# streamer45/streamkit

Hardware: AMD Instinct MI355X
Metric: real-time factor (audio-sec/wall-sec) Whisper-small Oneshot batch (higher is better)
Workload: dtype f16; 1 GPU; Whisper-small Oneshot batch, 64x30 s synthetic 16 kHz clips per GPU (configs[1]), greedy T=0 with the temperature ladder armed, random-init weights in GGML f16 container; precision=f16_mfma: f16 operands on v_mfma_f32_16x16x32_f16, f32 accumulate, clips_per_gpu=64, fallback_requested=0

## Files before the change

streamkit_amd/csrc/skw_kernels_f16.hip:

```cpp
#include "skw_dev_common.h"
#include <algorithm>
#include <atomic>
#include <type_traits>

typedef _Float16 f16x8 __attribute__((ext_vector_type(8)));
#ifndef SKW_VOCAB_W_AUX
#define SKW_VOCAB_W_AUX 0
#endif
#ifndef SKW_EPI_ST_NT
#define SKW_EPI_ST_NT 0
#endif
#ifndef SKW_EPI_RES_NT
#define SKW_EPI_RES_NT 0
#endif
#ifndef SKW_DEC_W_AUX
#define SKW_DEC_W_AUX 0
#endif
#define MFMA16X32(a, b, c) __builtin_amdgcn_mfma_f32_16x16x32_f16((a), (b), (c), 0, 0, 0)

typedef __attribute__((address_space(1))) const void* gptr_t;
typedef __attribute__((address_space(3))) void* lptr_t;

__device__ __forceinline__ int inv_kperm32(int p) { return ((p & 7) << 2) | ((p >> 3) & 3); }
template <int EPI> struct Epi16 {
// ... 105 lines not shown
            int gn = n0 + c; if (gn > a.N - 1) gn = a.N - 1;
            gB[i] = a.W + (long)gn * a.ldw + pchunk * 8;
        }
    };
    auto stage = [&](int buf, int kb) {
        char* base = lds + buf * (BM + BN) * 128;
        if (PROBE && (a.probe & 32)) {
#pragma unroll
            for (int i = 0; i < A_PIECES; ++i) __builtin_amdgcn_global_load_lds((gptr_t)(gA[i] + kb * 64), (lptr_t)(base + (wave * A_PIECES + i) * 1024), 16, 0, 2);
        } else {
#pragma unroll
            for (int i = 0; i < A_PIECES; ++i) __builtin_amdgcn_global_load_lds((gptr_t)(gA[i] + kb * 64), (lptr_t)(base + (wave * A_PIECES + i) * 1024), 16, 0, 0);
        }
        if (PROBE && (a.probe & 64)) {
#pragma unroll
            for (int i = 0; i < B_PIECES; ++i) __builtin_amdgcn_global_load_lds((gptr_t)(gB[i] + kb * 64), (lptr_t)(base + BM * 128 + (wave * B_PIECES + i) * 1024), 16, 0, 2);
        } else {
#pragma unroll
            for (int i = 0; i < B_PIECES; ++i) __builtin_amdgcn_global_load_lds((gptr_t)(gB[i] + kb * 64), (lptr_t)(base + BM * 128 + (wave * B_PIECES + i) * 1024), 16, 0, 0);
        }
    };
    const int fo0 = ((g ^ (r16 & 7)) << 4), fo1 = fo0 ^ 64;
    const int aoff = (wr * WTM + r16) * 128, boff = BM * 128 + (wc * WTN + r16) * 128;
    const int xoff = X_IS_M ? aoff : boff, yoff = X_IS_M ? boff : aoff;
    const int nk = a.K >> 6;
    const int x_lim = X_IS_M ? Mv : a.N, y_lim = X_IS_M ? a.N : a.M;
    int tile = blockIdx.x;
    if (tile >= nblk) return;
    int m0, n0; tile_origin(tile, m0, n0); tile_sources(m0, n0);
    stage(0, 0);
    for (;;) {
        asm volatile("s_waitcnt vmcnt(0)" ::: "memory");
        __syncthreads();
        f32x4 acc[TX][TY];
#pragma unroll
        for (int i = 0; i < TX; ++i)
#pragma unroll
            for (int j = 0; j < TY; ++j) acc[i][j] = (f32x4){0.f, 0.f, 0.f, 0.f};
        for (int kb = 0; kb < nk; ++kb) {
            const char* base = lds + (kb & 1) * (BM + BN) * 128;
            if (!PROBE) stage((kb + 1) & 1, min(kb + 1, nk - 1));
            else if (kb + 1 < nk && !(a.probe & 1)) stage((kb + 1) & 1, kb + 1);
#pragma unroll
            for (int kk = 0; kk < 2; ++kk) {
                if (PROBE && (a.probe & 2)) break;
                const int fo = kk ? fo1 : fo0;
                f16x8 fx[TX], fy[TY];
#pragma unroll
                for (int t = 0; t < TX; ++t) fx[t] = *(const f16x8*)(base + xoff + t * 2048 + fo);
#pragma unroll
                for (int t = 0; t < TY; ++t) fy[t] = *(const f16x8*)(base + yoff + t * 2048 + fo);
#pragma unroll
                for (int i = 0; i < TX; ++i)
#pragma unroll
                    for (int j = 0; j < TY; ++j) acc[i][j] = MFMA16X32(fx[i], fy[j], acc[i][j]);
            }
            if (kb + 1 < nk) { asm volatile("s_waitcnt vmcnt(0)" ::: "memory"); __syncthreads(); }
        }
        if (!PROBE) asm volatile("s_waitcnt vmcnt(0)" ::: "memory");
        __syncthreads();
        const int X0 = X_IS_M ? m0 : n0, Y0 = X_IS_M ? n0 : m0;
        tile += gridDim.x;
        const bool more = tile < nblk;
        if (more) { tile_origin(tile, m0, n0); tile_sources(m0, n0); if (!(PROBE && (a.probe & 1))) stage(0, 0); }
        if (!(PROBE && (a.probe & 4))) {
            constexpr bool F32OUT = Epi16Out<EPI>::F32OUT;
            constexpr int BX = X_IS_M ? BM : BN, BY = X_IS_M ? BN : BM, WTX = X_IS_M ? WTM : WTN, WTY = X_IS_M ? WTN : WTM;
            constexpr int ESZ = F32OUT ? 4 : 2, ROWB = BX * ESZ, CPR = ROWB / 16;
            constexpr int RP = ((BM + BN) * 128) / ROWB < BY ? ((BM + BN) * 128) / ROWB : BY;
            constexpr int NPASS = BY / RP, CE = 16 / ESZ;
            static_assert(BY % RP == 0 && (CPR & (CPR - 1)) == 0, "whole passes, power-of-two chunks per row");
            char* stg = lds + (BM + BN) * 128;
            float* bias_l = (float*)(lds + 2 * (BM + BN) * 128);
            const int wX = X_IS_M ? wr : wc, wY = X_IS_M ? wc : wr;
            const int div = X_IS_M ? a.Tpad : (a.n_ctx > 0 ? a.n_ctx : 1), org = X_IS_M ? X0 : Y0;
            const int qb = org / div, rb = org % div;
            {
                constexpr int NB = X_IS_M ? BY : BX;
                if (tid < NB) { const int pos = (X_IS_M ? Y0 : X0) + tid; const int f = (PERM && !X_IS_M) ? ((pos & ~31) | inv_kperm32(pos & 31)) : pos;
                bias_l[tid] = (a.bias && f < a.N) ? a.bias[f] : 0.0f; }
                __syncthreads();
            }
            for (int pass = 0; pass < NPASS; ++pass) {
                auto phase_a = [&](auto raw_tag) {
                    constexpr bool RAW = decltype(raw_tag)::value;
#pragma unroll
                for (int j = 0; j < TY; ++j) {
                    const int yl = wY * WTY + j * 16 + r16;
                    if ((wY * WTY + j * 16) / RP != pass) continue;
                    const int ylp = yl - pass * RP;
#pragma unroll
                    for (int i = 0; i < TX; ++i) {
                        const int xl = wX * WTX + i * 16 + 4 * g, p0 = X0 + xl;
                        float o[4];
                        const f32x4 bx = X_IS_M ? (f32x4){bias_l[yl], bias_l[yl], bias_l[yl], bias_l[yl]} : *(const f32x4*)(bias_l + xl);
#pragma unroll
                        for (int r = 0; r < 4; ++r) {
                            o[r] = RAW ? acc[i][j][r] : epi_value<EPI>(a, p0 + r, acc[i][j][r], bx[r]);
                            if (X_IS_M) { int key = rb + (((xl + r) & ~31) | inv_kperm32((xl + r) & 31)); if (key >= a.Tpad) key -= a.Tpad; if (key >= a.n_ctx) o[r] = 0.0f; }
                        }
                        const int ck = xl / CE;
                        char* dst = stg + ylp * ROWB + ((ck ^ (ylp & (CPR - 1))) << 4);
                        if (F32OUT) *(f32x4*)dst = (f32x4){o[0], o[1], o[2], o[3]};
                        else *(f16x4*)(dst + ((xl % CE) >= 4 ? 8 : 0)) = (f16x4){f2h(o[0]), f2h(o[1]), f2h(o[2]), f2h(o[3])};
                    }
                }
                };
                if (PROBE && (a.probe & 16)) phase_a(std::true_type{}); else phase_a(std::false_type{});
                __syncthreads();
                constexpr int NCH = RP * CPR / (NW * 64), BATCH = !F32OUT ? 2 : (NCH < 4 ? NCH : 4);
                static_assert((RP * CPR) % (NW * 64) == 0 && NCH % BATCH == 0, "whole chunks per thread");
#pragma unroll 1
                for (int c0 = 0; c0 < NCH; c0 += BATCH) {
                    long off[BATCH]; f32x4 opnd[BATCH]; int lofs[BATCH];
#pragma unroll
                    for (int u = 0; u < BATCH; ++u) {
                        const int cid = tid + (c0 + u) * NW * 64, ylp = cid / CPR, pc = cid % CPR, ck = pc ^ (ylp & (CPR - 1));
                        const int y = Y0 + pass * RP + ylp, px = X0 + ck * CE;
                        lofs[u] = ylp * ROWB + (pc << 4);
                        off[u] = (y >= y_lim || px >= x_lim || (PROBE && (a.probe & 8))) ? -1 : epi_chunk_offset<EPI>(a, y, px, pass * RP + ylp, ck * CE, qb, rb);
                        if (EPI == EPI_F32) opnd[u] = (a.res && off[u] >= 0) ? (SKW_EPI_RES_NT ? __builtin_nontemporal_load((const f32x4*)(a.res + (long)y * a.ldres + px))
                                                                                                : *(const f32x4*)(a.res + (long)y * a.ldres + px))
                                                                              : (f32x4){0.f, 0.f, 0.f, 0.f};
                        if (EPI == EPI_CONV2) { int i = rb + pass * RP + ylp; if (i >= a.n_ctx) i -= a.n_ctx;
                        opnd[u] = (off[u] >= 0) ? *(const f32x4*)(a.pe + (long)i * a.N + px) : (f32x4){0.f, 0.f, 0.f, 0.f}; }
                    }
#pragma unroll
                    for (int u = 0; u < BATCH; ++u) {
                        if (off[u] < 0) continue;
                        if (F32OUT) {
                            f32x4 v = *(const f32x4*)(stg + lofs[u]);
                            if (EPI == EPI_F32) { if (a.res) { v[0] = v[0] + opnd[u][0]; v[1] = v[1] + opnd[u][1]; v[2] = v[2] + opnd[u][2]; v[3] = v[3] + opnd[u][3]; } }
                            else { v[0] = opnd[u][0] + v[0]; v[1] = opnd[u][1] + v[1]; v[2] = opnd[u][2] + v[2]; v[3] = opnd[u][3] + v[3]; }
                            if (SKW_EPI_ST_NT) __builtin_nontemporal_store(v, (f32x4*)((float*)a.C + off[u])); else *(f32x4*)((float*)a.C + off[u]) = v;
                        } else { const u32x4 o16 = *(const u32x4*)(stg + lofs[u]); if (SKW_EPI_ST_NT) __builtin_nontemporal_store(o16, (u32x4*)((half_t*)a.C + off[u]));
                        else *(u32x4*)((half_t*)a.C + off[u]) = o16; }
                    }
                }
                __syncthreads();
            }
        }
        if (!more) break;
    }
}

static int skw_cur_device() { int dev = 0; if (hipGetDevice(&dev) != hipSuccess || dev < 0 || dev >= 64) dev = 0; return dev; }
static int skw_cu_count() {
    static std::atomic<int> n[64];
    const int dev = skw_cur_device(); int v = n[dev].load(std::memory_order_relaxed);
    if (!v) { hipDeviceProp_t p; v = (hipGetDeviceProperties(&p, dev) == hipSuccess && p.multiProcessorCount > 0) ? p.multiProcessorCount : 256; n[dev].store(v, std::memory_order_relaxed); }
    return v;
}
#define SKW_LDS_BARRIER() asm volatile("s_waitcnt lgkmcnt(0)\n\ts_barrier" ::: "memory")
template <int EPI, bool PROBE = false>
__global__ __launch_bounds__(256, 2) void k_gemm16w(SkwGemmArgs a) {
    constexpr int BM = 128, BN = 256, NW = 4, WTN = 64, TMT = BM / 16, TNT = WTN / 16, SLOT = BM * 128, NSLOT = 3, PARK = 32768;
    constexpr bool X_IS_M = Epi16<EPI>::X_IS_M, PERM = Epi16<EPI>::PERM;
    constexpr int TX = X_IS_M ? TMT : TNT, TY = X_IS_M ? TNT : TMT;
    constexpr int A_PIECES = BM / 8 / NW;
    __shared__ __attribute__((aligned(1024))) char lds[65536];
    const int tid = threadIdx.x, lane = tid & 63, wave = __builtin_amdgcn_readfirstlane(tid >> 6);
    const int Mv = X_IS_M ? (a.M / a.n_ctx) * a.Tpad : a.M;
    const int nbn = (a.N + BN - 1) / BN, nbm = (Mv + BM - 1) / BM, nblk = nbn * nbm;
    const int r16 = lane & 15, g = lane >> 4;
    const int prow = lane >> 3, pchunk = (lane & 7) ^ prow;
    const int nk = a.K >> 6, nk32 = a.K >> 5, nstrip = a.N >> 4;
    const half_t* gA[A_PIECES];
    unsigned woff[TNT];
    const int ng = a.wgroups > 1 ? a.wgroups : 1, ngn = nbn / ng, mparts = 8 / ng, mp = (nbm + mparts - 1) / mparts;
    const int nwalk = ng > 1 ? 8 * mp * ngn : nblk;
    auto tile_origin = [&](int tile, int& m0, int& n0) {
        if (ng > 1) {
            const int x = tile & 7, y = tile >> 3, gsel = x % ng, part = x / ng;
            const int m = part * mp + y / ngn;
            m0 = m < min(nbm, (part + 1) * mp) ? m * BM : -1; n0 = (gsel * ngn + y % ngn) * BN;
            return;
        }
        int q = nblk >> 3, r = nblk & 7, x = tile & 7, y = tile >> 3;
        const int bid = (x < r ? x * (q + 1) : r * (q + 1) + (x - r) * q) + y;
        m0 = (bid / nbn) * BM; n0 = (bid % nbn) * BN;
    };
    auto tile_sources = [&](int m0, int n0) {
#pragma unroll
        for (int i = 0; i < A_PIECES; ++i) {
            int c = (wave * A_PIECES + i) * 8 + prow; if (X_IS_M && PERM) c = (c & ~31) | inv_kperm32(c & 31);
            int gm = m0 + c;
            if (PROBE && (a.probe & 32768)) gm = c;
            if (X_IS_M) { const int b = gm / a.Tpad, key = gm % a.Tpad; gm = min(b, a.M / a.n_ctx - 1) * a.n_ctx + min(key, a.n_ctx - 1); }
            if (gm > a.M - 1) gm = a.M - 1;
            const long off = a.a_rows_per_batch ? (long)(gm / a.a_rows_per_batch) * a.a_batch_stride + (long)(gm % a.a_rows_per_batch) * a.lda : (long)gm * a.lda;
            gA[i] = a.A + off + pchunk * 8;
        }
#pragma unroll
        for (int t = 0; t < TNT; ++t) {
            int s = (n0 + wave * WTN + 16 * t) >> 4; if (s > nstrip - 1) s = nstrip - 1;
            woff[t] = (unsigned)(s * nk32) * 1024u + lane * 16;
        }
    };
    auto stage = [&](int slot, int kb) {
        char* base = lds + slot * SLOT;
#pragma unroll
        for (int i = 0; i < A_PIECES; ++i) __builtin_amdgcn_global_load_lds((gptr_t)(gA[i] + kb * 64), (lptr_t)(base + (wave * A_PIECES + i) * 1024), 16, 0, 0);
    };
    auto loadw = [&](f16x8 (&w)[TNT], int kb32) {
#pragma unroll
        for (int t = 0; t < TNT; ++t) asm volatile("global_load_dwordx4 %0, %1, %2" : "=v"(w[t]) : "v"(woff[t] + (unsigned)kb32 * 1024u), "s"(a.Wf) : "memory");
    };
    const int fo0 = ((g ^ (r16 & 7)) << 4), fo1 = fo0 ^ 64;
    const int aoff = r16 * 128;
    const int x_lim = X_IS_M ? Mv : a.N, y_lim = X_IS_M ? a.N : a.M;
    constexpr int BIAS_OFF = NSLOT * SLOT, BIAS_MAX = (65536 - BIAS_OFF) / 4;
    const bool bias_lds = a.N <= BIAS_MAX;
    if (bias_lds) {
        float* bl = (float*)(lds + BIAS_OFF);
        for (int p = tid; p < a.N; p += 256) { const int f = (PERM && !X_IS_M) ? ((p & ~31) | inv_kperm32(p & 31)) : p; bl[p] = a.bias ? a.bias[f] : 0.0f; }
        SKW_LDS_BARRIER();
    }
    for (int tile = blockIdx.x; tile < nwalk; tile += gridDim.x) {
        int m0, n0; tile_origin(tile, m0, n0);
        if (m0 < 0) continue;
        tile_sources(m0, n0);
        f16x8 w0[TNT], w1[TNT];
        stage(0, 0);
        stage(1, min(1, nk - 1));
        loadw(w0, 0);
        stage(2, min(2, nk - 1));
        loadw(w1, 1);
        f32x4 acc[TX][TY];
#pragma unroll
        for (int i = 0; i < TX; ++i)
#pragma unroll
            for (int j = 0; j < TY; ++j) acc[i][j] = (f32x4){0.f, 0.f, 0.f, 0.f};
        asm volatile("s_waitcnt vmcnt(16)" ::: "memory");
        __builtin_amdgcn_s_barrier();
        f16x8 lo[4], hi[4];
        auto rd = [&](f16x8 (&f)[4], const char* base, int t0, int fo) {
#pragma unroll
            for (int t = 0; t < 4; ++t) f[t] = *(const f16x8*)(base + aoff + (t0 + t) * 2048 + fo);
        };
        auto mm = [&](const f16x8 (&f)[4], const f16x8 (&w)[TNT], int t0, f16x8 (&nf)[4], const char* nb, int nt0, int nfo) {
            if (PROBE && (a.probe & 4096)) { asm volatile("" :: "v"(f[0]), "v"(f[3]), "v"(w[0])); rd(nf, nb, nt0, nfo); return; }
#pragma unroll
            for (int t = 0; t < 4; ++t)
#pragma unroll
                for (int q = 0; q < TNT; ++q) {
                    if (X_IS_M) acc[t0 + t][q] = MFMA16X32(f[t], w[q], acc[t0 + t][q]);
                    else acc[q][t0 + t] = MFMA16X32(w[q], f[t], acc[q][t0 + t]);
                    if (t == 0 && q == 0) { __builtin_amdgcn_sched_barrier(0); rd(nf, nb, nt0, nfo); __builtin_amdgcn_sched_barrier(0); }
                }
        };
        rd(lo, lds, 0, fo0);
        for (int kb = 0; kb < nk; ++kb) {
            const char* base = lds + (kb % NSLOT) * SLOT;
            const char* nbase = lds + ((kb + 1) % NSLOT) * SLOT;
            asm volatile("s_waitcnt vmcnt(8)" : "+v"(w0[0]), "+v"(w0[1]), "+v"(w0[2]), "+v"(w0[3]) :: "memory");
            mm(lo, w0, 0, hi, base, 4, fo0);
            __builtin_amdgcn_sched_barrier(0);
            mm(hi, w0, 4, lo, base, 0, fo1);
            if (!(PROBE && (a.probe & 8192))) loadw(w0, min(2 * kb + 2, nk32 - 1));
            __builtin_amdgcn_sched_barrier(0);
            asm volatile("s_waitcnt vmcnt(4)" : "+v"(w1[0]), "+v"(w1[1]), "+v"(w1[2]), "+v"(w1[3]) :: "memory");
            mm(lo, w1, 0, hi, base, 4, fo1);
            __builtin_amdgcn_sched_barrier(0);
            asm volatile("s_waitcnt lgkmcnt(0)\n\ts_barrier" : "+v"(hi[0]), "+v"(hi[1]), "+v"(hi[2]), "+v"(hi[3]) :: "memory");
            if (!(PROBE && (a.probe & 16384))) stage(kb % NSLOT, min(kb + 3, nk - 1));
            mm(hi, w1, 4, lo, nbase, 0, fo0);
            if (!(PROBE && (a.probe & 8192))) loadw(w1, min(2 * kb + 3, nk32 - 1));
            __builtin_amdgcn_sched_barrier(0);
        }
        asm volatile("" :: "v"(lo[0]), "v"(lo[1]), "v"(lo[2]), "v"(lo[3]));
        asm volatile("s_waitcnt vmcnt(0)" : "+v"(w0[0]), "+v"(w0[1]), "+v"(w0[2]), "+v"(w0[3]), "+v"(w1[0]), "+v"(w1[1]), "+v"(w1[2]), "+v"(w1[3]) :: "memory");
        __syncthreads();
        const int X0 = X_IS_M ? m0 : n0, Y0 = X_IS_M ? n0 : m0;
        if (PROBE && (a.probe & 1024)) { asm volatile("" :: "v"(acc[0][0]), "v"(acc[TX - 1][TY - 1])); }
        else {
            constexpr bool F32OUT = Epi16Out<EPI>::F32OUT;
            constexpr int ESZ = F32OUT ? 4 : 2, CE = 16 / ESZ;
            constexpr int WX = X_IS_M ? BM : WTN, WY = X_IS_M ? WTN : BM;
            constexpr int RB = WX * ESZ, CPRW = RB / 16;
            constexpr int FILLB = 8192;
            constexpr int RH = FILLB / RB < WY ? FILLB / RB : WY, NFILL = WY / RH;
            constexpr int NCH = RH * CPRW / 64, TYF = RH / 16;
            static_assert(WY % RH == 0 && (RH * CPRW) % 64 == 0 && RH % 16 == 0, "whole fills");
            char* wl = lds + wave * FILLB;
            const int xw = X_IS_M ? 0 : wave * WTN, yw = X_IS_M ? wave * WTN : 0;
            const int div = X_IS_M ? a.Tpad : (a.n_ctx > 0 ? a.n_ctx : 1), org = X_IS_M ? X0 : Y0;
            const int qb = org / div, rb = org % div;
            constexpr bool FASTOFF = (EPI == EPI_HEADS_F16);
            const bool interior = FASTOFF && Y0 + BM <= y_lim && X0 + BN <= x_lim && rb + BM <= div;
            const bool has_pad = X_IS_M && (rb + BM > a.n_ctx);
            f32x4 bx[X_IS_M ? 1 : TX]; float by[X_IS_M ? TY : 1];
            const float* bl = (const float*)(lds + BIAS_OFF);
            if (!X_IS_M) {
#pragma unroll
                for (int i = 0; i < TX; ++i) {
                    const int p0 = X0 + xw + i * 16 + 4 * g;
                    if (bias_lds) bx[i] = (p0 < a.N) ? *(const f32x4*)(bl + p0) : (f32x4){0.f, 0.f, 0.f, 0.f};
                    else {
#pragma unroll
                        for (int r = 0; r < 4; ++r) { const int pos = p0 + r, f = PERM ? ((pos & ~31) | inv_kperm32(pos & 31)) : pos; bx[i][r] = (a.bias && f < a.N) ? a.bias[f] : 0.0f; }
                    }
                }
            } else {
#pragma unroll
                for (int j = 0; j < TY; ++j) { const int f = Y0 + yw + j * 16 + r16; by[j] = (f < a.N) ? (bias_lds ? bl[f] : (a.bias ? a.bias[f] : 0.0f)) : 0.0f; }
            }
#pragma unroll
            for (int fill = 0; fill < NFILL; ++fill) {
                f32x4 opnd[F32OUT ? NCH : 1];
                if (F32OUT) {
#pragma unroll
                    for (int u = 0; u < NCH; ++u) {
                        const int cid = lane + 64 * u, rho = cid / CPRW, pc = cid % CPRW, ck = pc ^ (rho & (CPRW - 1));
                        const int dy = yw + fill * RH + rho, y = Y0 + dy, px = X0 + xw + ck * CE;
                        const bool in = y < y_lim && px < x_lim && !(PROBE && (a.probe & 65536));
                        if (EPI == EPI_F32) opnd[u] = (a.res && in) ? *(const f32x4*)(a.res + (long)y * a.ldres + px) : (f32x4){0.f, 0.f, 0.f, 0.f};
                        if (EPI == EPI_CONV2) { int i = rb + dy; if (i >= a.n_ctx) i -= a.n_ctx;
                                                opnd[u] = in ? *(const f32x4*)(a.pe + (long)i * a.N + px) : (f32x4){0.f, 0.f, 0.f, 0.f}; }
                    }
                }
#pragma unroll
                for (int jj = 0; jj < TYF; ++jj) {
                    const int j = fill * TYF + jj, rho = jj * 16 + r16;
#pragma unroll
                    for (int i = 0; i < TX; ++i) {
                        const int xl = i * 16 + 4 * g;
                        float o[4];
#pragma unroll
                        for (int r = 0; r < 4; ++r) {
                            o[r] = epi_value<EPI>(a, 0, acc[i][j][r], X_IS_M ? by[j] : bx[i][r]);
                            if (X_IS_M && has_pad) { int key = rb + (((xl + r) & ~31) | inv_kperm32((xl + r) & 31)); if (key >= a.Tpad) key -= a.Tpad; if (key >= a.n_ctx) o[r] = 0.0f; }
                        }
                        const int ck = xl / CE;
                        char* dst = wl + rho * RB + ((ck ^ (rho & (CPRW - 1))) << 4);
                        if (F32OUT) *(f32x4*)dst = (f32x4){o[0], o[1], o[2], o[3]};
                        else *(f16x4*)(dst + ((((xl % CE) >= 4) != (((rho >> 3) & 1) != 0)) ? 8 : 0)) = (f16x4){f2h(o[0]), f2h(o[1]), f2h(o[2]), f2h(o[3])};
                    }
                }
                asm volatile("s_waitcnt lgkmcnt(0)" ::: "memory");
                __builtin_amdgcn_sched_barrier(0);
                constexpr int RS = 64 / CPRW;
                long off0 = 0; long ostep = 0;
                if (interior) {
                    const int rho = lane / CPRW, pc = lane % CPRW, ck = pc ^ (rho & (CPRW - 1)), dy = yw + fill * RH + rho, dx = xw + ck * CE;
                    off0 = epi_chunk_offset<EPI>(a, Y0 + dy, X0 + dx, dy, dx, qb, rb) - (long)ck * CE;
                    ostep = (long)RS * (EPI == EPI_HEADS_F16 ? 64 : a.ldc);
                }
#pragma unroll
                for (int u = 0; u < NCH; ++u) {
                    const int cid = lane + 64 * u, rho = cid / CPRW, pc = cid % CPRW, ck = pc ^ (rho & (CPRW - 1));
                    const int dy = yw + fill * RH + rho, dx = xw + ck * CE, y = Y0 + dy, px = X0 + dx;
                    long off;
                    if (interior) off = off0 + u * ostep + ck * CE;
                    else {
                        if (y >= y_lim || px >= x_lim) continue;
                        off = epi_chunk_offset<EPI>(a, y, px, dy, dx, qb, rb);
                    }
                    if (PROBE && (a.probe & 65536)) continue;
                    const char* src = wl + cid * 16;
                    if (F32OUT) {
                        f32x4 v = *(const f32x4*)src;
                        if (EPI == EPI_F32) { if (a.res) { v[0] = v[0] + opnd[u][0]; v[1] = v[1] + opnd[u][1]; v[2] = v[2] + opnd[u][2]; v[3] = v[3] + opnd[u][3]; } }
                        else { v[0] = opnd[u][0] + v[0]; v[1] = opnd[u][1] + v[1]; v[2] = opnd[u][2] + v[2]; v[3] = opnd[u][3] + v[3]; }
                        *(f32x4*)((float*)a.C + off) = v;
                    } else { u32x4 o16 = *(const u32x4*)src; if ((rho >> 3) & 1) o16 = (u32x4){o16[2], o16[3], o16[0], o16[1]}; *(u32x4*)((half_t*)a.C + off) = o16; }
                }
                if (fill + 1 < NFILL) asm volatile("s_waitcnt lgkmcnt(0)" ::: "memory");
            }
            SKW_LDS_BARRIER();
        }
    }
}
template <int EPI> static void launch_gemm16w(const SkwGemmArgs& a_in, hipStream_t s) {
    SkwGemmArgs a = a_in;
    const int Mv = Epi16<EPI>::X_IS_M ? (a.M / a.n_ctx) * a.Tpad : a.M;
    const int nbn_ = (a.N + 255) / 256, nbm_ = (Mv + 127) / 128;
    const int ng_env = skw_sw(SW_GEMM16W_NGROUPS);
    int ng = 1;
    if (ng_env > 1) ng = ng_env;
    else if (ng_env == 0 && !Epi16<EPI>::X_IS_M) { const double wb = 2.0 * a.N * a.K; while (ng < 8 && wb / ng > 2.6e6 && nbn_ % (2 * ng) == 0) ng *= 2; }
    if (ng > 1 && (nbn_ % ng || 8 % ng || Epi16<EPI>::X_IS_M)) ng = 1;
    a.wgroups = ng;
    const int nblk = ng > 1 ? 8 * ((nbm_ + 8 / ng - 1) / (8 / ng)) * (nbn_ / ng) : nbm_ * nbn_;
    const int slots = ((a.probe & 2048) ? 1 : 2) * (skw_cu_count() & ~7);
    if (a.probe) hipLaunchKernelGGL((k_gemm16w<EPI, true>), dim3(std::min(nblk, slots)), dim3(256), 0, s, a);
    else hipLaunchKernelGGL((k_gemm16w<EPI>), dim3(std::min(nblk, slots)), dim3(256), 0, s, a);
}
static bool gemm16w_ok(const SkwGemmArgs& a) {
    return skw_sw(SW_GEMM16W) && a.Wf && !(a.probe & 1023) && (a.K & 63) == 0 && (a.N & 15) == 0 && a.M >= 128;
}
bool skw_gemm16_takes_w(const SkwGemmArgs& a) { return gemm16w_ok(a); }
template <int EPI> static void launch_gemm16(const SkwGemmArgs& a_in, hipStream_t s) {
    const int Mv = Epi16<EPI>::X_IS_M ? (a_in.M / a_in.n_ctx) * a_in.Tpad : a_in.M;
    const bool big = Mv >= 256 && a_in.N >= 256 && Mv % 256 == 0 && a_in.N % 256 == 0;
    const int cus = skw_cu_count() & ~7;
    const SkwGemmArgs& a = a_in;
    if (big && a.probe) { const int nblk = ((Mv + 255) / 256) * ((a.N + 255) / 256);
    hipLaunchKernelGGL((k_gemm16<EPI, 256, 256, 2, 4, true>), dim3(std::min(nblk, cus)), dim3(512), 0, s, a); }
    else if (big) { const int nblk = ((Mv + 255) / 256) * ((a.N + 255) / 256); hipLaunchKernelGGL((k_gemm16<EPI, 256, 256, 2, 4>), dim3(std::min(nblk, cus)), dim3(512), 0, s, a); }
    else { const int nblk = ((Mv + 127) / 128) * ((a.N + 127) / 128); hipLaunchKernelGGL((k_gemm16<EPI, 128, 128, 2, 2>), dim3(std::min(nblk, 2 * cus)), dim3(256), 0, s, a); }
}
void skw_gemm16(const SkwGemmArgs& a, hipStream_t s) {
    if (gemm16w_ok(a)) {
        switch (a.epi) {
            case EPI_F32: launch_gemm16w<EPI_F32>(a, s); return;
            case EPI_F16_KPERM: launch_gemm16w<EPI_F16_KPERM>(a, s); return;
            case EPI_GELU_F16_KPERM: launch_gemm16w<EPI_GELU_F16_KPERM>(a, s); return;
            case EPI_GELU_F16_KPERM_ROWPAD: launch_gemm16w<EPI_GELU_F16_KPERM_ROWPAD>(a, s); return;
            case EPI_CONV2: launch_gemm16w<EPI_CONV2>(a, s); return;
            case EPI_HEADS_F16: launch_gemm16w<EPI_HEADS_F16>(a, s); return;
            case EPI_VT_F16: launch_gemm16w<EPI_VT_F16>(a, s); return;
            case EPI_F16_PLAIN: launch_gemm16w<EPI_F16_PLAIN>(a, s); return;
            default: break;
        }
    }
    switch (a.epi) {
        case EPI_F32: launch_gemm16<EPI_F32>(a, s); break;
        case EPI_F16_KPERM: launch_gemm16<EPI_F16_KPERM>(a, s); break;
        case EPI_GELU_F16_KPERM: launch_gemm16<EPI_GELU_F16_KPERM>(a, s); break;
        case EPI_GELU_F16_KPERM_ROWPAD: launch_gemm16<EPI_GELU_F16_KPERM_ROWPAD>(a, s); break;
        case EPI_CONV2: launch_gemm16<EPI_CONV2>(a, s); break;
        case EPI_HEADS_F16: launch_gemm16<EPI_HEADS_F16>(a, s); break;
        case EPI_VT_F16: launch_gemm16<EPI_VT_F16>(a, s); break;
        case EPI_F16_PLAIN: launch_gemm16<EPI_F16_PLAIN>(a, s); break;
    }
}

#define A16_QB 128
struct SkwXPrefill { const int* row0; const int* nq; const int* slot; long ldq; long k_seq_stride; long ldk; int frag; int ofrag_k; const int* slot_k; int out_rows; };
template <bool XP, int OCC = 2, bool VARK = false>
__global__ __launch_bounds__(256, OCC) void k_attn_encoder16(const half_t* Qh, const half_t* Kh, const half_t* Vt, half_t* out, long ld_out,
                                                           int H, int n_ctx, int Tpad, float kq_scale, int qblocks, SkwXPrefill xp) {
    __shared__ __attribute__((aligned(1024))) char lds[2][2][64 * 128];
    const int tid = threadIdx.x, lane = tid & 63, wave = __builtin_amdgcn_readfirstlane(tid >> 6);
    const int nblk = gridDim.x; int bid = blockIdx.x;
    { int q = nblk >> 3, r = nblk & 7, x = bid & 7, y = bid >> 3; bid = (x < r ? x * (q + 1) : r * (q + 1) + (x - r) * q) + y; }
    long bh = bid / qblocks; const int qb = bid % qblocks;
    const int b = (int)(bh / H), h = (int)(bh % H);
    int n_q = n_ctx; long qrow0 = 0;
    if (XP) { n_q = xp.nq[b]; qrow0 = xp.row0[b]; if (qb * A16_QB >= n_q) return; bh = (long)xp.slot[b] * H + h; }
    int n_k = n_ctx;
    if constexpr (VARK) { n_k = min(n_ctx, max(1, xp.slot_k[XP ? xp.slot[b] : b])); if (!XP) { n_q = n_k; if (qb * A16_QB >= n_q) return; } }
    const int q0 = qb * A16_QB + wave * 32;
    const int r16 = lane & 15, g = lane >> 4;
    f16x8 qf[2][2];
#pragma unroll
    for (int qt = 0; qt < 2; ++qt) {
        int qi = q0 + qt * 16 + r16; if (qi > n_q - 1) qi = n_q - 1;
        const half_t* qp = XP ? Qh + (qrow0 + qi) * xp.ldq + h * 64 + g * 8 : Qh + (bh * Tpad + qi) * 64 + g * 8;
        qf[qt][0] = *(const f16x8*)qp; qf[qt][1] = *(const f16x8*)(qp + 32);
    }
    const long krow = XP ? xp.ldk : 64;
    const bool frag = XP && xp.frag;
    __amdgpu_buffer_rsrc_t rk = frag ? __builtin_amdgcn_make_buffer_rsrc((void*)(Kh + (long)xp.slot[b] * xp.k_seq_stride + (long)h * (Tpad >> 4) * 1024), 0, (unsigned)((Tpad >> 4) * 2048), 0x00020000)
                              : XP ? __builtin_amdgcn_make_buffer_rsrc((void*)(Kh + (long)xp.slot[b] * xp.k_seq_stride + h * 64), 0, (unsigned)((((long)n_ctx - 1) * krow + 64) * 2), 0x00020000)
                                   : __builtin_amdgcn_make_buffer_rsrc((void*)(Kh + bh * Tpad * 64), 0, (unsigned)(Tpad * 64 * 2), 0x00020000);
    __amdgpu_buffer_rsrc_t rv = __builtin_amdgcn_make_buffer_rsrc((void*)(Vt + bh * 64 * Tpad), 0, (unsigned)(64 * Tpad * 2), 0x00020000);
    unsigned st_lds[2], st_ldsk[2], st_k[2], st_v[2]; int st_vkey[2];
#pragma unroll
    for (int i = 0; i < 2; ++i) {
        const int c = tid + 256 * i, row = c >> 3, pos = c & 7;
        st_lds[i] = (unsigned)(row * 128 + ((pos ^ (row & 7)) << 4));
        st_ldsk[i] = (unsigned)(row * 128 + ((pos ^ ((row >> 1) & 6)) << 4));
        st_k[i] = (unsigned)((row * krow + pos * 8) * 2);
        st_v[i] = (unsigned)((row * Tpad + pos * 8) * 2);
        if (frag) {
            const int r = row & 15;
            st_k[i] = (unsigned)((((row >> 4) * 2 + (pos >> 2)) * 1024) + (4 * (r & 3) + (r >> 2) + 16 * (pos & 3)) * 16);
            st_v[i] = (unsigned)((((pos >> 2) * 4 + (row >> 4)) * 1024) + (r + 16 * (pos & 3)) * 16);
        }
        st_vkey[i] = pos * 8;
    }
    const int nkb = VARK ? (n_k + 63) >> 6 : (Tpad + 63) >> 6;
    const int kappa = 4 * (r16 & 3) + (r16 >> 2);
    const int k_off = kappa * 128, k_sw = (r16 & 3) << 1, v_off = r16 * 128, v_sw = r16 & 7;
    u32x4 sk[2], sv[2];
    auto load_k = [&](int kb) {
#pragma unroll
        for (int i = 0; i < 2; ++i) sk[i] = __builtin_amdgcn_raw_buffer_load_b128(rk, st_k[i] + (unsigned)kb * (frag ? 8192u : (unsigned)(krow * 128)), 0, 0);
    };
    auto load_v = [&](int kb) {
#pragma unroll
        for (int i = 0; i < 2; ++i) sv[i] = __builtin_amdgcn_raw_buffer_load_b128(rv, (kb * 64 + st_vkey[i] < Tpad) ? st_v[i] + (unsigned)kb * (frag ? 8192u : 128u) : 0x7fffff00u, 0, 0);
    };
    auto store_k = [&](int buf) {
#pragma unroll
        for (int i = 0; i < 2; ++i) *(u32x4*)(&lds[buf][0][st_ldsk[i]]) = sk[i];
    };
    auto store_v = [&](int buf) {
#pragma unroll
        for (int i = 0; i < 2; ++i) *(u32x4*)(&lds[buf][1][st_lds[i]]) = sv[i];
    };
    auto scores = [&](const char* kbase, int kt, f32x4& s0, f32x4& s1) {
        const f16x8 k0 = *(const f16x8*)(kbase + kt * 2048 + k_off + ((g ^ k_sw) << 4));
        const f16x8 k1 = *(const f16x8*)(kbase + kt * 2048 + k_off + (((4 | g) ^ k_sw) << 4));
        s0 = MFMA16X32(k0, qf[0][0], ((f32x4){0.f, 0.f, 0.f, 0.f})); s1 = MFMA16X32(k0, qf[1][0], ((f32x4){0.f, 0.f, 0.f, 0.f}));
        s0 = MFMA16X32(k1, qf[0][1], s0); s1 = MFMA16X32(k1, qf[1][1], s1);
    };
    const float c1 = kq_scale * 1.44269504088896341f;
    float m0 = -INFINITY, m1 = -INFINITY;
    f32x4 lacc0 = {0.f, 0.f, 0.f, 0.f}, lacc1 = {0.f, 0.f, 0.f, 0.f};
    f16x8 ones; for (int e = 0; e < 8; ++e) ones[e] = (half_t)1.0f;
    f32x4 oacc[2][4];
#pragma unroll
    for (int qt = 0; qt < 2; ++qt)
#pragma unroll
        for (int ct = 0; ct < 4; ++ct) oacc[qt][ct] = (f32x4){0.f, 0.f, 0.f, 0.f};
    load_k(0); load_v(0); store_k(0); store_v(0); __syncthreads();
    for (int kb = 0; kb < nkb; ++kb) {
        const char* kbase = &lds[kb & 1][0][0]; const char* vbase = &lds[kb & 1][1][0];
        if (kb + 1 < nkb) { load_k(kb + 1); load_v(kb + 1); }
        f32x4 s0[4], s1[4];
        float bm0 = -INFINITY, bm1 = -INFINITY;
#pragma unroll
        for (int kt = 0; kt < 4; ++kt) {
            scores(kbase, kt, s0[kt], s1[kt]);
            if (kb == nkb - 1) {
#pragma unroll
                for (int r = 0; r < 4; ++r) if (kb * 64 + kt * 16 + 4 * r + g >= n_k) { s0[kt][r] = -INFINITY; s1[kt][r] = -INFINITY; }
            }
#pragma unroll
            for (int r = 0; r < 4; ++r) { bm0 = fmaxf(bm0, s0[kt][r]); bm1 = fmaxf(bm1, s1[kt][r]); }
        }
        bm0 = skw_rows_max_f32(bm0); bm1 = skw_rows_max_f32(bm1);
        if (__builtin_amdgcn_ballot_w64(bm0 > m0 || bm1 > m1)) {
            const float n0 = fmaxf(m0, bm0), n1 = fmaxf(m1, bm1);
            const float a0 = __builtin_amdgcn_exp2f((m0 - n0) * c1), a1 = __builtin_amdgcn_exp2f((m1 - n1) * c1);
#pragma unroll
            for (int ct = 0; ct < 4; ++ct)
#pragma unroll
                for (int r = 0; r < 4; ++r) { oacc[0][ct][r] *= a0; oacc[1][ct][r] *= a1; }
            for (int r = 0; r < 4; ++r) { lacc0[r] *= a0; lacc1[r] *= a1; }
            m0 = n0; m1 = n1;
        }
        const float mc0 = m0 * c1, mc1 = m1 * c1;
        f16x8 p0[2], p1[2];
#pragma unroll
        for (int kt = 0; kt < 4; ++kt)
#pragma unroll
// ... 438 lines not shown
```

Before: 11210 x real-time.

## Prefetch next tile's A and W during epilogue in persistent f16 weight GEMM

The persistent k_gemm16w kernel now uses four LDS slots and dynamic shared memory (76 KB). While the current tile's epilogue runs, it issues the next tile's A stages into two spare slots and its first weight fragments. This hides the pipeline-fill latency between consecutive tiles. The cost is more LDS per block, which may limit two-blocks-per-CU occupancy, plus extra register pressure and more complex waitcnt ordering. Lane-derived values are also recomputed from mbcnt to cut live registers.

```diff
diff --git a/streamkit_amd/csrc/skw_kernels_f16.hip b/streamkit_amd/csrc/skw_kernels_f16.hip
--- a/streamkit_amd/csrc/skw_kernels_f16.hip
+++ b/streamkit_amd/csrc/skw_kernels_f16.hip
@@ -281,18 +281,26 @@
     return v;
 }
 #define SKW_LDS_BARRIER() asm volatile("s_waitcnt lgkmcnt(0)\n\ts_barrier" ::: "memory")
+#define SKW_GEMM16W_LDS (4 * 16384 + 12288)
 template <int EPI, bool PROBE = false>
 __global__ __launch_bounds__(256, 2) void k_gemm16w(SkwGemmArgs a) {
-    constexpr int BM = 128, BN = 256, NW = 4, WTN = 64, TMT = BM / 16, TNT = WTN / 16, SLOT = BM * 128, NSLOT = 3, PARK = 32768;
+    constexpr int BM = 128, BN = 256, NW = 4, WTN = 64, TMT = BM / 16, TNT = WTN / 16, SLOT = BM * 128, NSLOT = 4, LDSB = SKW_GEMM16W_LDS;
     constexpr bool X_IS_M = Epi16<EPI>::X_IS_M, PERM = Epi16<EPI>::PERM;
     constexpr int TX = X_IS_M ? TMT : TNT, TY = X_IS_M ? TNT : TMT;
     constexpr int A_PIECES = BM / 8 / NW;
-    __shared__ __attribute__((aligned(1024))) char lds[65536];
-    const int tid = threadIdx.x, lane = tid & 63, wave = __builtin_amdgcn_readfirstlane(tid >> 6);
+    extern __shared__ __attribute__((aligned(1024))) char lds[];
+    const int tid = threadIdx.x, wave = __builtin_amdgcn_readfirstlane(tid >> 6);
     const int Mv = X_IS_M ? (a.M / a.n_ctx) * a.Tpad : a.M;
     const int nbn = (a.N + BN - 1) / BN, nbm = (Mv + BM - 1) / BM, nblk = nbn * nbm;
-    const int r16 = lane & 15, g = lane >> 4;
-    const int prow = lane >> 3, pchunk = (lane & 7) ^ prow;
+    auto uni = [](int v) { asm volatile("" : "+s"(v)); return v; };
+    int r16, g, prow, pchunk, fo0, fo1, aoff;
+    auto lane_now = [&]() { int l; asm volatile("v_mbcnt_lo_u32_b32 %0, -1, 0\n\tv_mbcnt_hi_u32_b32 %0, -1, %0" : "=v"(l)); return l; };
+    auto relane = [&]() {
+        const int l = lane_now();
+        r16 = l & 15; g = l >> 4; prow = l >> 3; pchunk = (l & 7) ^ prow;
+        fo0 = ((g ^ (r16 & 7)) << 4); fo1 = fo0 ^ 64; aoff = r16 * 128;
+    };
+    relane();
     const int nk = a.K >> 6, nk32 = a.K >> 5, nstrip = a.N >> 4;
     const half_t* gA[A_PIECES];
     unsigned woff[TNT];
@@ -300,30 +308,34 @@
     const int nwalk = ng > 1 ? 8 * mp * ngn : nblk;
     auto tile_origin = [&](int tile, int& m0, int& n0) {
         if (ng > 1) {
-            const int x = tile & 7, y = tile >> 3, gsel = x % ng, part = x / ng;
-            const int m = part * mp + y / ngn;
-            m0 = m < min(nbm, (part + 1) * mp) ? m * BM : -1; n0 = (gsel * ngn + y % ngn) * BN;
+            const int x = tile & 7, y = tile >> 3, ng_ = uni(ng), ngn_ = uni(ngn), gsel = x % ng_, part = x / ng_;
+            const int m = part * mp + y / ngn_;
+            m0 = m < min(nbm, (part + 1) * mp) ? m * BM : -1; n0 = (gsel * ngn_ + y % ngn_) * BN;
             return;
         }
         int q = nblk >> 3, r = nblk & 7, x = tile & 7, y = tile >> 3;
         const int bid = (x < r ? x * (q + 1) : r * (q + 1) + (x - r) * q) + y;
-        m0 = (bid / nbn) * BM; n0 = (bid % nbn) * BN;
-    };
-    auto tile_sources = [&](int m0, int n0) {
+        const int nbn_ = uni(nbn); m0 = (bid / nbn_) * BM; n0 = (bid % nbn_) * BN;
+    };
+    auto tile_sources_a = [&](int m0) {
+        const int tpad = uni(a.Tpad), rpb = uni(a.a_rows_per_batch);
 #pragma unroll
         for (int i = 0; i < A_PIECES; ++i) {
             int c = (wave * A_PIECES + i) * 8 + prow; if (X_IS_M && PERM) c = (c & ~31) | inv_kperm32(c & 31);
             int gm = m0 + c;
             if (PROBE && (a.probe & 32768)) gm = c;
-            if (X_IS_M) { const int b = gm / a.Tpad, key = gm % a.Tpad; gm = min(b, a.M / a.n_ctx - 1) * a.n_ctx + min(key, a.n_ctx - 1); }
+            if (X_IS_M) { const int b = gm / tpad, key = gm % tpad; gm = min(b, a.M / a.n_ctx - 1) * a.n_ctx + min(key, a.n_ctx - 1); }
             if (gm > a.M - 1) gm = a.M - 1;
-            const long off = a.a_rows_per_batch ? (long)(gm / a.a_rows_per_batch) * a.a_batch_stride + (long)(gm % a.a_rows_per_batch) * a.lda : (long)gm * a.lda;
+            const long off = rpb ? (long)(gm / rpb) * a.a_batch_stride + (long)(gm % rpb) * a.lda : (long)gm * a.lda;
             gA[i] = a.A + off + pchunk * 8;
         }
+    };
+    auto tile_sources_w = [&](int n0) {
+        const int l16 = lane_now() * 16;
 #pragma unroll
         for (int t = 0; t < TNT; ++t) {
             int s = (n0 + wave * WTN + 16 * t) >> 4; if (s > nstrip - 1) s = nstrip - 1;
-            woff[t] = (unsigned)(s * nk32) * 1024u + lane * 16;
+            woff[t] = (unsigned)(s * nk32) * 1024u + l16;
         }
     };
     auto stage = [&](int slot, int kb) {
@@ -335,33 +347,32 @@
 #pragma unroll
         for (int t = 0; t < TNT; ++t) asm volatile("global_load_dwordx4 %0, %1, %2" : "=v"(w[t]) : "v"(woff[t] + (unsigned)kb32 * 1024u), "s"(a.Wf) : "memory");
     };
-    const int fo0 = ((g ^ (r16 & 7)) << 4), fo1 = fo0 ^ 64;
-    const int aoff = r16 * 128;
     const int x_lim = X_IS_M ? Mv : a.N, y_lim = X_IS_M ? a.N : a.M;
-    constexpr int BIAS_OFF = NSLOT * SLOT, BIAS_MAX = (65536 - BIAS_OFF) / 4;
+    constexpr int BIAS_OFF = NSLOT * SLOT, BIAS_MAX = (LDSB - BIAS_OFF) / 4;
     const bool bias_lds = a.N <= BIAS_MAX;
     if (bias_lds) {
         float* bl = (float*)(lds + BIAS_OFF);
         for (int p = tid; p < a.N; p += 256) { const int f = (PERM && !X_IS_M) ? ((p & ~31) | inv_kperm32(p & 31)) : p; bl[p] = a.bias ? a.bias[f] : 0.0f; }
         SKW_LDS_BARRIER();
     }
-    for (int tile = blockIdx.x; tile < nwalk; tile += gridDim.x) {
-        int m0, n0; tile_origin(tile, m0, n0);
-        if (m0 < 0) continue;
-        tile_sources(m0, n0);
-        f16x8 w0[TNT], w1[TNT];
-        stage(0, 0);
-        stage(1, min(1, nk - 1));
-        loadw(w0, 0);
-        stage(2, min(2, nk - 1));
-        loadw(w1, 1);
+    auto next_real = [&](int t, int& m0, int& n0) { for (; t < nwalk; t += gridDim.x) { tile_origin(t, m0, n0); if (m0 >= 0) return t; } return nwalk; };
+    f16x8 w0[TNT], w1[TNT];
+    auto prefetch_a = [&](int m0) { tile_sources_a(m0); stage(2, 0); stage(3, min(1, nk - 1)); };
+    auto prefetch_w = [&](int n0) { tile_sources_w(n0); loadw(w0, 0); loadw(w1, 1); };
+    auto tile_start = [&](int m0) {
+        if (Epi16Out<EPI>::F32OUT) { asm volatile("" : "+v"(m0)); tile_sources_a(m0); }
+        stage(0, min(2, nk - 1));
+        asm volatile("s_waitcnt vmcnt(4)" : "+v"(w0[0]), "+v"(w0[1]), "+v"(w0[2]), "+v"(w0[3]), "+v"(w1[0]), "+v"(w1[1]), "+v"(w1[2]), "+v"(w1[3]) :: "memory");
+        __builtin_amdgcn_s_barrier();
+    };
+    int m0 = 0, n0 = 0, tile = next_real(blockIdx.x, m0, n0);
+    if (tile < nwalk) { prefetch_a(m0); prefetch_w(n0); tile_start(m0); }
+    while (tile < nwalk) {
         f32x4 acc[TX][TY];
 #pragma unroll
         for (int i = 0; i < TX; ++i)
 #pragma unroll
             for (int j = 0; j < TY; ++j) acc[i][j] = (f32x4){0.f, 0.f, 0.f, 0.f};
-        asm volatile("s_waitcnt vmcnt(16)" ::: "memory");
-        __builtin_amdgcn_s_barrier();
         f16x8 lo[4], hi[4];
         auto rd = [&](f16x8 (&f)[4], const char* base, int t0, int fo) {
 #pragma unroll
@@ -378,10 +389,10 @@
                     if (t == 0 && q == 0) { __builtin_amdgcn_sched_barrier(0); rd(nf, nb, nt0, nfo); __builtin_amdgcn_sched_barrier(0); }
                 }
         };
-        rd(lo, lds, 0, fo0);
+        rd(lo, lds + 2 * SLOT, 0, fo0);
         for (int kb = 0; kb < nk; ++kb) {
-            const char* base = lds + (kb % NSLOT) * SLOT;
-            const char* nbase = lds + ((kb + 1) % NSLOT) * SLOT;
+            const char* base = lds + ((kb + 2) % NSLOT) * SLOT;
+            const char* nbase = lds + ((kb + 3) % NSLOT) * SLOT;
             asm volatile("s_waitcnt vmcnt(8)" : "+v"(w0[0]), "+v"(w0[1]), "+v"(w0[2]), "+v"(w0[3]) :: "memory");
             mm(lo, w0, 0, hi, base, 4, fo0);
             __builtin_amdgcn_sched_barrier(0);
@@ -392,7 +403,7 @@
             mm(lo, w1, 0, hi, base, 4, fo1);
             __builtin_amdgcn_sched_barrier(0);
             asm volatile("s_waitcnt lgkmcnt(0)\n\ts_barrier" : "+v"(hi[0]), "+v"(hi[1]), "+v"(hi[2]), "+v"(hi[3]) :: "memory");
-            if (!(PROBE && (a.probe & 16384))) stage(kb % NSLOT, min(kb + 3, nk - 1));
+            if (!(PROBE && (a.probe & 16384))) stage((kb + 1) % NSLOT, min(kb + 3, nk - 1));
             mm(hi, w1, 4, lo, nbase, 0, fo0);
             if (!(PROBE && (a.probe & 8192))) loadw(w1, min(2 * kb + 3, nk32 - 1));
             __builtin_amdgcn_sched_barrier(0);
@@ -401,19 +412,25 @@
         asm volatile("s_waitcnt vmcnt(0)" : "+v"(w0[0]), "+v"(w0[1]), "+v"(w0[2]), "+v"(w0[3]), "+v"(w1[0]), "+v"(w1[1]), "+v"(w1[2]), "+v"(w1[3]) :: "memory");
         __syncthreads();
         const int X0 = X_IS_M ? m0 : n0, Y0 = X_IS_M ? n0 : m0;
-        if (PROBE && (a.probe & 1024)) { asm volatile("" :: "v"(acc[0][0]), "v"(acc[TX - 1][TY - 1])); }
+        const int ntile = next_real(tile + gridDim.x, m0, n0);
+        if (ntile < nwalk) prefetch_a(m0);
+        if (PROBE && (a.probe & 1024)) { asm volatile("" :: "v"(acc[0][0]), "v"(acc[TX - 1][TY - 1]));
+            if (ntile < nwalk) prefetch_w(n0);
+            if (ntile < nwalk) { asm volatile("s_waitcnt vmcnt(0)" : "+v"(w0[0]), "+v"(w0[1]), "+v"(w0[2]), "+v"(w0[3]), "+v"(w1[0]), "+v"(w1[1]), "+v"(w1[2]), "+v"(w1[3]) :: "memory"); } }
         else {
             constexpr bool F32OUT = Epi16Out<EPI>::F32OUT;
             constexpr int ESZ = F32OUT ? 4 : 2, CE = 16 / ESZ;
+            const int lane_t = lane_now();
+            const int lane = lane_t, r16 = lane & 15, g = lane >> 4;
             constexpr int WX = X_IS_M ? BM : WTN, WY = X_IS_M ? WTN : BM;
             constexpr int RB = WX * ESZ, CPRW = RB / 16;
-            constexpr int FILLB = 8192;
+            constexpr int FILLB = EPI == EPI_CONV2 ? 4096 : 8192;
             constexpr int RH = FILLB / RB < WY ? FILLB / RB : WY, NFILL = WY / RH;
             constexpr int NCH = RH * CPRW / 64, TYF = RH / 16;
             static_assert(WY % RH == 0 && (RH * CPRW) % 64 == 0 && RH % 16 == 0, "whole fills");
             char* wl = lds + wave * FILLB;
             const int xw = X_IS_M ? 0 : wave * WTN, yw = X_IS_M ? wave * WTN : 0;
-            const int div = X_IS_M ? a.Tpad : (a.n_ctx > 0 ? a.n_ctx : 1), org = X_IS_M ? X0 : Y0;
+            const int div = uni(X_IS_M ? a.Tpad : (a.n_ctx > 0 ? a.n_ctx : 1)), org = X_IS_M ? X0 : Y0;
             const int qb = org / div, rb = org % div;
             constexpr bool FASTOFF = (EPI == EPI_HEADS_F16);
             const bool interior = FASTOFF && Y0 + BM <= y_lim && X0 + BN <= x_lim && rb + BM <= div;
@@ -436,11 +453,12 @@
             }
 #pragma unroll
             for (int fill = 0; fill < NFILL; ++fill) {
+                int lane_f = lane; asm volatile("" : "+v"(lane_f));
                 f32x4 opnd[F32OUT ? NCH : 1];
                 if (F32OUT) {
 #pragma unroll
                     for (int u = 0; u < NCH; ++u) {
-                        const int cid = lane + 64 * u, rho = cid / CPRW, pc = cid % CPRW, ck = pc ^ (rho & (CPRW - 1));
+                        const int cid = lane_f + 64 * u, rho = cid / CPRW, pc = cid % CPRW, ck = pc ^ (rho & (CPRW - 1));
                         const int dy = yw + fill * RH + rho, y = Y0 + dy, px = X0 + xw + ck * CE;
                         const bool in = y < y_lim && px < x_lim && !(PROBE && (a.probe & 65536));
                         if (EPI == EPI_F32) opnd[u] = (a.res && in) ? *(const f32x4*)(a.res + (long)y * a.ldres + px) : (f32x4){0.f, 0.f, 0.f, 0.f};
@@ -467,17 +485,18 @@
                     }
                 }
                 asm volatile("s_waitcnt lgkmcnt(0)" ::: "memory");
+                if (fill == NFILL - 1 && ntile < nwalk) { __builtin_amdgcn_sched_barrier(0); prefetch_w(n0); }
                 __builtin_amdgcn_sched_barrier(0);
                 constexpr int RS = 64 / CPRW;
                 long off0 = 0; long ostep = 0;
                 if (interior) {
-                    const int rho = lane / CPRW, pc = lane % CPRW, ck = pc ^ (rho & (CPRW - 1)), dy = yw + fill * RH + rho, dx = xw + ck * CE;
+                    const int rho = lane_f / CPRW, pc = lane_f % CPRW, ck = pc ^ (rho & (CPRW - 1)), dy = yw + fill * RH + rho, dx = xw + ck * CE;
                     off0 = epi_chunk_offset<EPI>(a, Y0 + dy, X0 + dx, dy, dx, qb, rb) - (long)ck * CE;
                     ostep = (long)RS * (EPI == EPI_HEADS_F16 ? 64 : a.ldc);
                 }
 #pragma unroll
                 for (int u = 0; u < NCH; ++u) {
-                    const int cid = lane + 64 * u, rho = cid / CPRW, pc = cid % CPRW, ck = pc ^ (rho & (CPRW - 1));
+                    const int cid = lane_f + 64 * u, rho = cid / CPRW, pc = cid % CPRW, ck = pc ^ (rho & (CPRW - 1));
                     const int dy = yw + fill * RH + rho, dx = xw + ck * CE, y = Y0 + dy, px = X0 + dx;
                     long off;
                     if (interior) off = off0 + u * ostep + ck * CE;
@@ -496,8 +515,12 @@
                 }
                 if (fill + 1 < NFILL) asm volatile("s_waitcnt lgkmcnt(0)" ::: "memory");
             }
-            SKW_LDS_BARRIER();
-        }
+            asm volatile("s_waitcnt vmcnt(0)" : "+v"(w0[0]), "+v"(w0[1]), "+v"(w0[2]), "+v"(w0[3]), "+v"(w1[0]), "+v"(w1[1]), "+v"(w1[2]), "+v"(w1[3]) :: "memory");
+        }
+        SKW_LDS_BARRIER();
+        relane();
+        if (ntile < nwalk) tile_start(m0);
+        tile = ntile;
     }
 }
 template <int EPI> static void launch_gemm16w(const SkwGemmArgs& a_in, hipStream_t s) {
@@ -512,8 +535,13 @@
     a.wgroups = ng;
     const int nblk = ng > 1 ? 8 * ((nbm_ + 8 / ng - 1) / (8 / ng)) * (nbn_ / ng) : nbm_ * nbn_;
     const int slots = ((a.probe & 2048) ? 1 : 2) * (skw_cu_count() & ~7);
-    if (a.probe) hipLaunchKernelGGL((k_gemm16w<EPI, true>), dim3(std::min(nblk, slots)), dim3(256), 0, s, a);
-    else hipLaunchKernelGGL((k_gemm16w<EPI>), dim3(std::min(nblk, slots)), dim3(256), 0, s, a);
+    static std::atomic<bool> once[64];
+    { const int dev = skw_cur_device(); if (!once[dev].load(std::memory_order_acquire)) {
+        hipFuncSetAttribute((const void*)k_gemm16w<EPI, true>, hipFuncAttributeMaxDynamicSharedMemorySize, SKW_GEMM16W_LDS);
+        hipFuncSetAttribute((const void*)k_gemm16w<EPI>, hipFuncAttributeMaxDynamicSharedMemorySize, SKW_GEMM16W_LDS);
+        once[dev].store(true, std::memory_order_release); } }
+    if (a.probe) hipLaunchKernelGGL((k_gemm16w<EPI, true>), dim3(std::min(nblk, slots)), dim3(256), SKW_GEMM16W_LDS, s, a);
+    else hipLaunchKernelGGL((k_gemm16w<EPI>), dim3(std::min(nblk, slots)), dim3(256), SKW_GEMM16W_LDS, s, a);
 }
 static bool gemm16w_ok(const SkwGemmArgs& a) {
     return skw_sw(SW_GEMM16W) && a.Wf && !(a.probe & 1023) && (a.K & 63) == 0 && (a.N & 15) == 0 && a.M >= 128;
```

After: 11260 x real-time, median of 5. About the same (+0.4%).
